# StavrosOrf/EV2Gym

Measured on AMD Instinct MI355X. Metric: env-steps/sec (envs x chargers x steps); % HBM roofline, higher is better.
Workload: dtype f64; 1 GPU; cfg2: V2GProfitPlusLoads, 50 chargers, 1 transformer, uniform[-1,1] actions; envs_per_gpu=4096, scenario_pool_per_gpu=32768, scenario_pool_order=sorted by busy window inside every window of envs_per_gpu scenarios, chargers=50, transformers=1, steps_per_episode=112, obs_dim=162, soc_log=True, launch=persistent, actor=none

## Files before the change

### ev2gym_amd/csrc/ev2g_host.hip

```cpp
#include <hip/hip_runtime.h>

#include <algorithm>
#include <cmath>
#include <cstdio>
#include <cstring>
#include <array>
#include <map>
#include <string>
#include <vector>

#include "../../include/ev2g.h"
#include "ev2g_device.h"
#include "ev2g_load_host.h"
#include "ev2g_step_v2.h"
#include "ev2g_step_wave.h"
#include "ev2g_step_big.h"
#include "ev2g_mlp.h"
#include "ev2g_comm.h"
#include "ev2g_refill.h"
#include "ev2g_heuristic.h"
#include "ev2g_link.h"
#include "ev2g_grid.h"
#include "ev2g_wrap.h"
#include "ev2g_ac.h"
// ... 124 lines not shown
    std::string big_reason;
    size_t lds_big = 0;
    BigArgs big_args{};
    bool no_full = false, no_wide = false;
    bool no_strided = false;
    std::map<ClsKey, int> cls_map;
    ClsRec *d_cls_rec = nullptr;
    std::vector<double> cs_vk_host;
    std::vector<int> cs_ph_host;
    std::vector<double> cs_imax_host;
    int load_gen = 0;
    int last_spec = -1;
    double *d_stats_inl = nullptr;
    const char *inl_shape_reason = "";
    bool inl_stats = false, no_inl_stats = false;
    int last_stats_route = -1;
    const char *inl_reason = "";
    const char *stats_reason = "";
    const char *general_reason = "";
    bool pow2_dt = false;
    std::string kernel_name;
    std::string fallback_reason;
    int current_step = 0;
    long long state_epoch = 0;
    size_t lds_bytes = 0;
    hipEvent_t ev0s[EV2G_EV_RING] = {}, ev1s[EV2G_EV_RING] = {};
    int ev_slot = 0;
    bool ev_valid[EV2G_EV_RING] = {};
    unsigned fused_attr_mask = 0;
    long long ev_calls = 0;
// ... 171 lines not shown
    if (h->own_stream) (void)hipStreamDestroy(h->stream);
    delete h;
}

int ev2g_n_envs(const ev2g_handle *h) { return h ? h->E : 0; }
int ev2g_n_ports(const ev2g_handle *h) { return h ? h->P : 0; }
int ev2g_obs_dim(const ev2g_handle *h) { return h ? h->D : 0; }
int ev2g_n_steps(const ev2g_handle *h) { return h ? h->T : 0; }
int ev2g_current_step(const ev2g_handle *h) { return h ? h->current_step : 0; }
const char *ev2g_kernel_name(const ev2g_handle *h) { return (h && h->loaded) ? h->kernel_name.c_str() : ""; }
const char *ev2g_fallback_reason(const ev2g_handle *h) { return (h && h->loaded) ? h->fallback_reason.c_str() : ""; }
const char *ev2g_big_kernel_reason(const ev2g_handle *h) { return (h && h->loaded) ? h->big_reason.c_str() : ""; }
int ev2g_last_launch_specialisation(const ev2g_handle *h) { return (h && h->loaded) ? h->last_spec : -1; }
int ev2g_last_stats_route(const ev2g_handle *h) { return (h && h->loaded) ? h->last_stats_route : -1; }
const char *ev2g_last_stats_reason(const ev2g_handle *h) { return (h && h->loaded && h->last_stats_route == 0) ? h->stats_reason : ""; }
const char *ev2g_last_launch_general_reason(const ev2g_handle *h) { return (h && h->loaded && h->last_spec == 0) ? h->general_reason : ""; }

static const char *kStatNames[EV2G_N_STATS] = {
    "total_ev_served", "total_profits", "total_energy_charged", "total_energy_discharged",
    "average_user_satisfaction", "power_tracker_violation", "tracking_error", "energy_tracking_error",
    "energy_user_satisfaction", "std_energy_user_satisfaction", "min_energy_user_satisfaction",
    "total_steps_min_emergency_battery_capacity_violation", "total_transformer_overload",
    "battery_degradation", "battery_degradation_calendar", "battery_degradation_cycling", "total_reward"};
const char *ev2g_stat_name(int i) { return (i >= 0 && i < EV2G_N_STATS) ? kStatNames[i] : ""; }

int ev2g_reset_ex(ev2g_handle *h, double *obs, int64_t scenario_offset);

static bool stats_pair(const ev2g_handle *h) {
    const long long per_scn = h->sess_cap > 0 ? (long long)h->sess_cap : (h->S + h->M - 1) / std::max(h->M, 1);
    return (h->sess_cap > 0 ? per_scn <= 48 : h->S <= (long long)h->M * 24) && h->C <= 32;
// ... 7 lines not shown
    s.E = E; s.M = M; s.T = T; s.C = C; s.npc = npc; s.P = P; s.R = R; s.D = D; s.ND = std::max(p.ND, 1); s.dt = p.dt;
    s.reward_kind = h->cfg.reward_kind; s.state_kind = sk; s.flags = h->cfg.flags; s.cost_kind = h->cfg.cost_kind; s.n_lut = p.n_lut;
    s.het = p.het ? 1 : 0;
    h->block = p.het ? 0 : (P <= 256) ? 256 : (P <= 512) ? 512 : (P <= 1024) ? 1024 : 0;
    const int blk = h->block ? h->block : EV2G_BLOCK;
    s.G = std::max(1, blk / P);
    s.G = std::min(s.G, E);
    h->fallback_reason.clear();
    if (P < 2 || P > 64) h->fallback_reason = "ports per env outside 2..64";
    else if (R != 1) h->fallback_reason = "more than one transformer";
    else if (npc != 1) h->fallback_reason = "multi-port chargers";
    if (p.het) h->fallback_reason = "chargers with different port counts (topology file)";
    h->wave_path = h->fallback_reason.empty();
    h->no_full = sw.no_full; h->no_wide = sw.no_wide; h->last_spec = -1;
    h->no_strided = sw.no_strided;
    h->no_inl_stats = sw.no_inl_stats; h->inl_stats = false; h->last_stats_route = -1; h->inl_reason = "no step launch since the scenarios were loaded";
    h->state_epoch += 1;
    if (h->wave_path) {
        const unsigned long long lim = 1ull << 32;
        const unsigned long long biggest = std::max({(unsigned long long)E * P * 8, (unsigned long long)E * D * 8,
                                                     (unsigned long long)M * (T + 1) * 60 * 8, (unsigned long long)p.SD * sizeof(SessRec),
                                                     (unsigned long long)M * T * 64, (unsigned long long)E * T * 8 * 3, (unsigned long long)M * P * 8, (unsigned long long)E * P * sizeof(PortLine),
                                                     (h->cfg.flags & EV2G_FLAG_LOG_SOC) ? (unsigned long long)E * T * P * 8 : 0ull,
                                                     (h->cfg.flags & EV2G_FLAG_LOG_CS_HISTORY) ? (unsigned long long)T * E * C * 8 : 0ull});
        if (biggest >= lim) { h->wave_path = false; h->fallback_reason = "an array of the batch reaches 4 GiB (32-bit byte offsets)"; }
    }
    if (h->wave_path) {
        h->wave_epw = 64 / P; h->wave_es = P;
        s.G = (EV2G_WAVE_BLOCK / 64) * h->wave_epw;
    }
// ... 245 lines not shown
    EV2G_SETP(v2p.ss_afap, h->d_ss_afap);
    int ex = 0;
    v2p.pow2_dt = (std::frexp(h->scn.sixty_over_dt, &ex) == 0.5 && h->scn.sixty_over_dt * h->scn.dt_over_60 == 1.0) ? 1 : 0;
    h->pow2_dt = v2p.pow2_dt != 0;
    return upload(h, h->st_allocs, &v2p, 1, &h->d_v2p);
}

static int load_decide_inl_stats(ev2g_handle *h) {
    h->d_stats_inl = nullptr;
    const char *why = "";
    if (h->no_inl_stats) why = "EV2G_NO_INLAUNCH_STATS is set";
    else if (!h->wave_path || !(h->cfg.flags & EV2G_FLAG_LOG_SOC)) why = "the step kernel is not ev2g_step_wave with the SoC log";
    else if (h->wave_epw != 1 || stats_pair(h)) why = "several envs per wavefront (the in-launch phase computes one env per wavefront, like the statistics kernel at this shape)";
    else if (h->lds_bytes < ev2g_inl_stats_lds_bytes()) why = "the step kernel's LDS is smaller than the phase's blocks";
    h->inl_shape_reason = why;
    if (!why[0]) {
        int rc = 0;
        if ((rc = dalloc(h, h->st_allocs, (size_t)h->E * EV2G_N_STATS, &h->d_stats_inl))) return rc;
        double *p = h->d_stats_inl;
        HIPCHK(h, hipMemcpy((char *)h->d_v2p + offsetof(V2P, stats_inl), &p, sizeof p, hipMemcpyHostToDevice));
    }
    return EV2G_OK;
}

int ev2g_load_scenarios(ev2g_handle *h, const ev2g_scenario_batch *b) {
    if (!h || !b) return fail(h, EV2G_ERR_ARG, "ev2g_load_scenarios: null argument");
    (void)hipSetDevice(h->device);
    const LoadSwitches sw = load_switches_from_env();
    LoadPlan plan;
    V2P v2p;
// ... 107 lines not shown
    io.reward = r.reward.p; io.r_stride = r.reward.stride;
    io.done = r.done.p; io.d_stride = r.done.stride;
    io.mask = r.mask.p; io.m_stride = r.mask.stride;
    io.scn_off = (int)h->scn_off;
    io.scn_stride = (auto_reset == EV2G_AUTO_RESET_NEXT) ? h->E % h->M : 0;
    io.step0 = (int)step0;
    io.log_soc = (h->cfg.flags & EV2G_FLAG_LOG_SOC) ? 1 : 0;
    io.act32 = r.actions.p ? nullptr : h->extras.actions_f32;
    io.obs32 = (h->extras.obs_f32 && h->extras.obs_f32_step_stride == 0) ? h->extras.obs_f32 : nullptr;
    return io;
}

static int launch_steps(ev2g_handle *h, const StepIO &io, int t0, int k, int auto_reset) {
    const DevScn &s = h->scn;
    h->inl_stats = false; h->inl_reason = "the step kernel is not ev2g_step_wave"; h->state_epoch += 1;
    if (h->wave_path) {
        const long long lim = 1ll << 32;
        const ev2g_step_extras &x = h->extras;
        if (io.a_stride * 8 >= lim || io.o_stride * 8 >= lim || io.r_stride * 8 >= lim || io.d_stride >= lim || io.m_stride >= lim ||
            x.cost_step_stride * 8 >= lim || x.obs_f32_step_stride * 4 >= lim || io.a_stride < 0 || io.o_stride < 0 || io.r_stride < 0 ||
            io.d_stride < 0 || io.m_stride < 0 || x.cost_step_stride < 0 || x.obs_f32_step_stride < 0)
            return fail(h, EV2G_ERR_ARG, "ev2g_step_n: a step stride is negative or reaches 4 GiB (unsupported by the fast-path kernel)");
        const V2P *pp = (const V2P *)h->d_v2p;
        const DevState &st = h->st;
        const FusedArgs fa0{};
        const WaveArgs wa{s.P, s.T, s.E, s.D, s.M, st.slab_port, st.slab_port_slice, st.hist,
                    st.env_acc, s.cs_pack, (char *)st.line, h->d_step_tab, (char *)st.port_dyn, s.dict, h->wave_epw, h->wave_es};
        const bool f64io = io.actions && io.obs && !x.obs_f32, f32io = !io.actions && io.act32 && !io.obs && io.obs32;
        const bool full0 = (f64io || f32io) && io.reward && io.done && io.mask && !x.cost && !(h->cfg.flags & EV2G_FLAG_LOG_CS_HISTORY) &&
                           !auto_reset && t0 + k <= s.T && std::min(s.reward_kind, 3) != 3 && !h->no_full;
        const bool wide0 = full0 && (h->cfg.flags & EV2G_FLAG_LOG_SOC) && s.P >= 3 && !h->no_wide &&
                           s.P >= (s.state_kind == EV2G_STATE_PUBLIC_PST ? 3 : (s.state_kind == EV2G_STATE_V2G_PROFIT_MAX_LOADS ? 30 : 10));
        const bool strided = io.o_stride != 0 || io.r_stride != 0 || io.d_stride != 0 || io.m_stride != 0;
        const bool str3 = strided && wide0 && f64io && !h->no_strided;
        const bool full = full0 && (!strided || str3), wide = wide0 && full;
        h->last_spec = full ? (str3 ? 3 : (wide ? 2 : 1)) : 0;
        {
            const char *why = "";
            if (!full) {
                if (h->no_full) why = "EV2G_NO_FULL is set (or the batch has more than 4094 efficiency tables)";
                else if (std::min(s.reward_kind, 3) == 3) why = "the reward function is one of the eight selected at run time (only the shipped configs' three are compiled in)";
                else if (h->cfg.flags & EV2G_FLAG_LOG_CS_HISTORY) why = "EV2G_FLAG_LOG_CS_HISTORY (charger histories)";
                else if (x.cost) why = "a cost buffer is registered (ev2g_set_step_extras)";
                else if (auto_reset) why = "auto_reset";
                else if (!(io.reward && io.done && io.mask)) why = "a reward / done / mask output is NULL";
                else if (!(f64io || f32io)) why = "the observation / action buffers are neither the float64 pair nor the float32 hand-over pair (e.g. obs NULL, or a float32 observation copy next to the float64 one)";
                else if (strided) why = "an output step stride is not 0 (strided outputs keep the specialisation only with float64 observations, EV2G_FLAG_LOG_SOC and an env wide enough for the wide instantiation)";
                else why = "the launch would run past the episode end";
            }
            h->general_reason = why;
        }
// ... 370 lines not shown
static bool fused_eligible(const ev2g_handle *h, const ev2g_mlp *m) {
    const DevScn &s = h->scn;
    const bool pst = s.state_kind == EV2G_STATE_PUBLIC_PST;
    return h->wave_path && s.P >= 3 && s.P <= 64 && std::min(s.reward_kind, 3) != 3 && (h->cfg.flags & EV2G_FLAG_LOG_SOC) &&
           !(h->cfg.flags & EV2G_FLAG_LOG_CS_HISTORY) && !h->extras.cost && !h->no_full && !h->no_wide && (pst || (s.D & 1) == 0) &&
           m->s16_ks1 == (pst ? 2 : 6) && m->s16_nt1 == 25 && m->s16_nt2 == 19 && m->s16_nt3 == (pst ? 2 : 4) &&
           (m->s16_nw == 1 || (m->s16_nw == 2 && !std::getenv("EV2G_NO_FUSED_F32"))) &&
           !std::getenv("EV2G_NO_FUSED");
}
static int launch_fused(ev2g_handle *h, const ev2g_mlp *m, int k, const float *obs0, Rows<float> obs, Rows<float> act, Rows<double> reward,
                        Rows<uint8_t> done, Rows<uint8_t> mask) {
    const DevScn &s = h->scn;
    const DevState &st = h->st;
    const long long lim = 1ll << 32;
    h->inl_stats = false; h->inl_reason = "the last launch was a policy-in-the-loop segment (ev2g_rollout / ev2g_collect)"; h->state_epoch += 1;
    if (obs.stride * 4 >= lim || act.stride * 4 >= lim || reward.stride * 8 >= lim || done.stride >= lim || mask.stride >= lim || obs.stride < 0 ||
        act.stride < 0 || reward.stride < 0 || done.stride < 0 || mask.stride < 0)
        return fail(h, EV2G_ERR_ARG, "ev2g_collect / ev2g_rollout: a step stride is negative or reaches 4 GiB");
    StepIO io = make_io(h, StepRows{{nullptr, act.stride}, {nullptr, obs.stride}, reward, done, mask}, 0, 0);
    io.act32 = act.p; io.obs32 = obs.p;
    const int ae = (s.state_kind == EV2G_STATE_PUBLIC_PST && s.P <= 32 && m->s16_nw == 1) ? 2 : 1;
    const WaveArgs wa{s.P, s.T, s.E, s.D, s.M, st.slab_port, st.slab_port_slice, st.hist, st.env_acc, s.cs_pack, (char *)st.line, h->d_step_tab, (char *)st.port_dyn, s.dict, ae, ae == 1 ? s.P : 32};
    FusedArgs fa{};
    fa.m = m->dev; fa.obs0 = obs0;
    const V2P *pp = (const V2P *)h->d_v2p;
    const int nwf = m->s16_nw;
    const size_t lds = ev2g_fused_lds_bytes(ae, nwf);
    const dim3 grid((s.E + 16 * ae - 1) / (16 * ae)), block(EV2G_FUSED_BLOCK);
    const int t0 = h->current_step;
#define EV2G_FUSED_CASE(SK, RK)                                                                                                            \
// ... 1348 lines not shown
```

### ev2gym_amd/csrc/ev2g_load_host.h

```cpp
#pragma once
#include <algorithm>
#include <array>
#include <cmath>
#include <cstdlib>
#include <cstring>
#include <map>
#include <string>
#include <utility>
#include <vector>

#include "../../include/ev2g.h"
#include "ev2g_records.h"

struct LoadSwitches {
    long long pool_session_cap = 0;
    bool no_full = false, no_wide = false, no_strided = false;
    bool no_inl_stats = false;
    bool kernel_v2 = false;
    bool no_dict = false;
    bool no_big = false;
};
inline LoadSwitches load_switches_from_env() {
    LoadSwitches sw;
    if (const char *e = std::getenv("EV2G_POOL_SESSION_CAP")) sw.pool_session_cap = std::atoll(e);
    sw.no_full = std::getenv("EV2G_NO_FULL") != nullptr;
    sw.no_wide = std::getenv("EV2G_NO_WIDE") != nullptr;
    sw.no_strided = std::getenv("EV2G_NO_STRIDED") != nullptr;
    sw.no_inl_stats = std::getenv("EV2G_NO_INLAUNCH_STATS") != nullptr;
    const char *kn = std::getenv("EV2G_KERNEL");
    sw.kernel_v2 = kn && std::string(kn) == "v2";
    sw.no_dict = std::getenv("EV2G_NO_DICT") != nullptr;
    sw.no_big = std::getenv("EV2G_NO_BIG") != nullptr;
    return sw;
}

typedef std::array<uint64_t, 11> ClsKey;
inline int cls_find_or_add(std::map<ClsKey, int> &map, std::vector<ClsRec> &tab, const ClsRec &c) {
    ClsKey k;
    const double f[11] = {c.pacmax, c.tsm, c.gate_ch, c.B, c.rB, c.v, c.rv, c.gate_dis, c.minB, c.emerg, c.pdismax};
    std::memcpy(k.data(), f, sizeof f);
    auto it = map.find(k);
    if (it != map.end()) return it->second;
    if (map.size() >= EV2G_CLS_CAP) return -1;
// ... 372 lines not shown
```

### ev2gym_amd/csrc/ev2g_step_v2.h

```cpp
#pragma once
#include "ev2g_device.h"

#ifdef EV2G_PHASE_TIMING
#define PT_DECL unsigned long long pt_last = __builtin_readcyclecounter(); unsigned long long pt_acc[18] = {0,0,0,0,0,0,0,0,0,0,0,0,0,0,0,0,0,0}; unsigned long long pt_cur[8] = {0,0,0,0,0,0,0,0};
#define PT_MARK(i) { unsigned long long n_ = __builtin_readcyclecounter(); pt_cur[i] += n_ - pt_last; pt_last = n_; }
#define PT_STEP_END(empty) { const int o_ = (empty) ? 8 : 0; for (int i_ = 0; i_ < 8; i_++) { pt_acc[o_ + i_] += pt_cur[i_]; pt_cur[i_] = 0; } pt_acc[16 + ((empty) ? 1 : 0)] += 1; }
#ifndef EV2G_PT_TID
#define EV2G_PT_TID 0
#endif
#define PT_FLUSH if (threadIdx.x == EV2G_PT_TID && S->dbg) { for (int i_ = 0; i_ < 8; i_++) pt_acc[i_] += pt_cur[i_]; for (int i_ = 0; i_ < 18; i_++) S->dbg[(size_t)blockIdx.x * 18 + i_] += pt_acc[i_]; }
#elif defined(EV2G_PHASE_MARKERS)
#define PT_DECL
#define PT_MARK(i) asm volatile("; PHASE_MARK " #i);
#define PT_STEP_END(empty)
#define PT_FLUSH
#else
#define PT_DECL
#define PT_MARK(i)
#define PT_STEP_END(empty)
#define PT_FLUSH
#endif

__device__ __forceinline__ void lds_barrier() { asm volatile("s_waitcnt lgkmcnt(0)\n\ts_barrier" ::: "memory"); }

// ... 96 lines not shown
    EV2G_GP(const double) head_tab;
    EV2G_GP(const SessRec) rec; EV2G_GP(const SessTail) tail; EV2G_GP(const int) ss_lut;
    EV2G_GP(const SessDyn) sess_dyn; EV2G_GP(const ClsRec) cls_rec;
    EV2G_GP(PortLine) line;
    EV2G_GP(double) cs_sat_sum; EV2G_GP(int) cs_served;
    EV2G_GP(double) cs_profits; EV2G_GP(double) cs_e_ch; EV2G_GP(double) cs_e_dis;
    EV2G_GP(double) cs_power_hist; EV2G_GP(double) cs_cur_hist; EV2G_GP(double) cs_power_now; EV2G_GP(double) cs_cur_now;
    EV2G_GP(double) env_acc; EV2G_GP(int) env_fault;
    EV2G_GP(double) hist; EV2G_GP(double) tr_power_now;
    EV2G_GP(double) sess_final_cap; EV2G_GP(double) port_energy; EV2G_GP(double) port_current;
    EV2G_GP(double) soc_log; EV2G_GP(double) sess_abs_e;
    EV2G_GP(unsigned long long) dbg;
    EV2G_GP(const int) scn_sess; EV2G_GP(const int) scn_sess_end; EV2G_GP(const int) ss_slot; EV2G_GP(const int) ss_tarr; EV2G_GP(const int) ss_tdep;
    EV2G_GP(const double) ss_B; EV2G_GP(const double) ss_afap;
    EV2G_GP(double) stats_inl;
    EV2G_GP(double) x_cost; long long x_c_stride;
    EV2G_GP(float) x_obs32; long long x_o32_stride;
    EV2G_GP(const float) x_act32;
};

inline void ev2g_v2_fill_params(V2P &p, const DevScn &s, const DevState &st) {
    p.E = s.E; p.M = s.M; p.cost_kind = s.cost_kind; p.T = s.T; p.C = s.C; p.npc = s.npc; p.P = s.P; p.R = s.R; p.D = s.D; p.G = s.G; p.dt = s.dt;
    p.reward_kind = s.reward_kind; p.state_kind = s.state_kind; p.n_lut = s.n_lut;
    p.sixty_over_dt = s.sixty_over_dt; p.dt_over_60 = s.dt_over_60;
    p.rdt = 1.0 / (double)s.dt; p.dt_fdiv = fabs(fma((double)s.dt, p.rdt, -1.0)) <= 0x1p-54 ? 1 : 0;
    EV2G_SETP(p.x_cost, (double *)nullptr); EV2G_SETP(p.x_obs32, (float *)nullptr); EV2G_SETP(p.x_act32, (const float *)nullptr);
    p.x_c_stride = 0; p.x_o32_stride = 0;
    p.pow2_dt = 0; EV2G_SETP(p.head_tab, (const double *)nullptr);
    EV2G_SETP(p.step_tab, (const double *)nullptr);
    EV2G_SETP(p.slab_port, st.slab_port); p.slab_port_slice = st.slab_port_slice;
    EV2G_SETP(p.slab_hist, st.slab_hist); EV2G_SETP(p.slab_sess, st.slab_sess);
    p.sess_slice = (unsigned long long)(st.sess_abs_e ? (st.sess_abs_e - st.slab_sess) : 0) * 8ull;
#define CPS(f) EV2G_SETP(p.f, s.f);
#define CPT(f) EV2G_SETP(p.f, st.f);
    CPS(slot_cs) CPS(slot_port) CPS(slot_obs) CPS(cs_slot0) CPS(tr_seg) CPS(tr_obs) CPS(port_first) CPS(port_first_win)
    CPS(cs_imax) CPS(cs_imin) CPS(cs_dmin) CPS(cs_dmax_abs) CPS(cs_maxp) CPS(cs_minp)
    CPS(price_ch) CPS(price_dis) CPS(setpoint) CPS(tr_infl) CPS(tr_solar) CPS(tr_base) CPS(tr_maxp) CPS(tr_minp)
    CPS(win_tab) CPS(lut) CPS(rec) CPS(tail) CPS(ss_lut) CPS(sess_dyn) CPS(cls_rec)
    CPS(scn_sess) CPS(scn_sess_end) CPS(ss_slot) CPS(ss_tarr) CPS(ss_tdep) CPS(ss_B)
    EV2G_SETP(p.ss_afap, (const double *)nullptr); EV2G_SETP(p.stats_inl, (double *)nullptr);
    CPT(line) CPT(cs_sat_sum) CPT(cs_served)
    CPT(cs_profits) CPT(cs_e_ch) CPT(cs_e_dis) CPT(cs_power_hist) CPT(cs_cur_hist) CPT(cs_power_now) CPT(cs_cur_now)
    CPT(env_acc) CPT(env_fault) CPT(hist) CPT(tr_power_now)
    CPT(sess_final_cap) CPT(port_energy) CPT(port_current) CPT(soc_log) CPT(sess_abs_e) CPT(dbg)
#undef CPS
#undef CPT
}

__host__ __device__ inline size_t ev2g_v2_lds_bytes(int NS, int NT, int G, int R) {
    return sizeof(double) * ((size_t)(EV2G_NQ + 7) * NS + (size_t)EV2G_NQ * NT + (size_t)EV2G_NQ * G + (size_t)NT +
                             (size_t)G * 9) +
           sizeof(int) * (6 * (size_t)NS + 2 * (size_t)R + 1 + 4);
}

#define V2C(x, c) (SPEC ? (c) : (x))
// ... 581 lines not shown
```

### ev2gym_amd/csrc/ev2g_step_wave.h

```cpp
#pragma once
#include <type_traits>
#include "ev2g_step_v2.h"
#include "ev2g_mlp.h"

#define EV2G_WAVE_BLOCK 256

__host__ __device__ inline size_t ev2g_wave_lds_bytes(int envs_per_group, int block = EV2G_WAVE_BLOCK) {
    const size_t NS = (size_t)block;
    return sizeof(double) * (EV2G_NQ * (NS + 8) + 7 * NS + 7 * (size_t)envs_per_group + 4 * 64) + sizeof(int) * (6 * NS + 8);
}
#define EV2G_INL_STATS_NK 12
#define EV2G_INL_STATS_LK 16
__host__ __device__ inline size_t ev2g_inl_stats_lds_bytes(int block = EV2G_WAVE_BLOCK) { return (size_t)block * EV2G_INL_STATS_LK * sizeof(double); }
#define EV2G_FUSED_BLOCK 1024
#define EV2G_FUSED_SX 200
#define EV2G_FUSED_RING 10
#define EV2G_FUSED_RING2 7

#define EV2G_FUSED_SXF 196
#define EV2G_FUSED_RINGF 4
__host__ __device__ inline size_t ev2g_fused_lds_bytes(int envs_per_wave = 1, int weight_terms = 1) {
    if (weight_terms > 1)
        return ev2g_wave_lds_bytes(EV2G_FUSED_BLOCK / 64 * envs_per_wave, EV2G_FUSED_BLOCK) + (size_t)16 * EV2G_FUSED_SXF * 4;
    return ev2g_wave_lds_bytes(EV2G_FUSED_BLOCK / 64 * envs_per_wave, EV2G_FUSED_BLOCK) + (size_t)16 * EV2G_FUSED_SX * 2 + (size_t)(25 + 19 + 4) * 16 * 4;
// ... 125 lines not shown
    float *lbias = (float *)(bufX + 16 * EV2G_FUSED_SX);
    float *act_lds = (float *)s_amps;
    uint16_t *bufH1 = (uint16_t *)stage, *bufH2 = bufH1 + 16 * AE * MC::SH1;
    constexpr int FSXF = EV2G_FUSED_SXF;
    float *bufXf = (float *)(cnt + 8);
    static_assert(NWF == 1 || (3 * 16 * MC::SH1 * 2 <= 5 * RS * 8 && EV2G_NQ == 8 && FKS1 * 32 <= 256), "the input rows' bf16 terms live in staging rows 5..7, behind H1's three copies");
    static_assert(NWF == 1 || (FKS1 * 32 + 4 <= FSXF && (3 * MC::SH1 + 2 * MC::SH2) * 16 * 2 <= EV2G_NQ * (EV2G_FUSED_BLOCK + 8) * 8 && MC::SH2 * 16 * 2 <= 16 * FSXF * 4), "float32 policy buffers");
    static_assert(AE * MC::SX <= EV2G_FUSED_SX && MC::NB <= (25 + 19 + 4) * 16 && 16 * AE * (MC::SH1 + MC::SH2) * 2 <= EV2G_NQ * (EV2G_FUSED_BLOCK + 8) * 8, "policy buffers");
    constexpr int ACT_AS = (AE == 1) ? 128 : 64;
    const int tid = threadIdx.x, wv = tid >> 6, lane = tid & 63;
    const bool log_soc = WIDE ? true : (S->soc_log != nullptr);
    const bool log_cs = FULL ? false : (S->cs_profits != nullptr);
    const double dtd = (double)S->dt, sixty_over_dt = S->sixty_over_dt, dt_over_60 = S->dt_over_60;
    const bool pow2_dt = S->pow2_dt != 0;

    const int elw = lane / ES;
    const int q = (ACT && AE == 1) ? lane : lane - elw * ES;
    const int e = (ACT && AE == 1) ? e0 + wv : e0 + wv * EPW + elw;
    const bool valid = (elw < EPW) && (q < P) && (e < E);
    const bool hcopy = ACT && AE == 1 && !valid && e < E && lane < 32;
    const int g = valid ? e * P + q : 0;
    const int ocol = (SK == 1) ? 3 + 3 * q : (SK == 0 ? 62 + 2 * q : 22 + 2 * q);
    const int cs = valid ? q : 0;
    int t = t0;
    const bool head = valid && q == 0;
    const int elg = wv * EPW + elw;
    const int arow = (AE == 1) ? wv : min(elg, 16 * AE - 1);
    auto xput2 = [&](int col, float a, float b) __attribute__((always_inline)) {
        if (NWF > 1) *(float2 *)(bufXf + arow * FSXF + col) = make_float2(a, b);
        else *(uint32_t *)(bufX + arow * FSX + col) = ev2g_pack_bf16(a, b);
// ... 183 lines not shown
        d2v pf_h0 = {0.0, 0.0}, pf_h1 = {0.0, 0.0};
        constexpr int NHEAD = (SK == 1) ? 0 : (SK == 0 ? 60 : 20);
        constexpr int NPAIR = NHEAD / 2;
        if (!out) {
        } else if (SK == 1) {
            pf_ob0 = ldg32_nt<double>(S->step_tab, eT64 + (unsigned)min(sstep, T - 1) * 64u + 40u);
        } else {
            const unsigned h8 = FULL ? hb_head + (unsigned)sstep * (unsigned)(NHEAD * 8) : (unsigned)((scn * (T + 1) + sstep) * NHEAD) * 8u;
            pf_h0 = ldg32_nt<d2v>(S->head_tab, h8 + (unsigned)min(q_l, NPAIR - 1) * 16u);
            if (!WIDE && P < NPAIR) pf_h1 = ldg32_nt<d2v>(S->head_tab, h8 + (unsigned)min(q_l + P, NPAIR - 1) * 16u);
        }
        bool occ = false;
        double cap_before = 0.0;
        int ta_a = EV2G_INT_MAX, td_a = -1;
        const bool wave_live = !FULL || EPW != 1 || __ballot(valid && ((r_ta <= t && t <= r_td) || r_ta == sstep)) != 0ull;
        if (valid && wave_live) {
            int ta = FULL ? r_ta : s_ta[tid_l], td = FULL ? r_td : s_td[tid_l];
            double cap_b = s_cap[tid_l], c_thr = s_cst[0 * 64 + q_l], c_dmin = s_cst[1 * 64 + q_l];
            asm volatile("s_waitcnt lgkmcnt(0)" : "+v"(ta), "+v"(td), "+v"(cap_b), "+v"(c_thr), "+v"(c_dmin));
            ta_a = ta; td_a = td;
            occ = (ta <= t) && (t <= td);
            if (log_soc && occ) cap_before = cap_b;
            double a = occ ? a_cur : 0.0;
            a = (a > 1.0) ? 1.0 : ((a < -1.0) ? -1.0 : a);
            const double n5 = rint(a * 100000.0), q5 = n5 * (1.0 / 100000.0);
            const double x = fma(fma(-q5, 100000.0, n5), 1.0 / 100000.0, q5);
            const double ac = x * c_imax, ad = x * c_dmaxabs;
            const double amps_c = (ac < c_thr) ? 0.0 : ac, amps_d = (ad > c_dmin - 0.01) ? c_dmin : ad;
            const double amps = (x > 0.0) ? amps_c : ((x < 0.0) ? amps_d : 0.0);
            s_amps[tid_l] = amps;
// ... 15 lines not shown
            static_assert(offsetof(SessRec, B) == 40 && offsetof(SessRec, rB) == 48 && offsetof(SessRec, cap0) == 112 && offsetof(SessRec, potc) == 120 && sizeof(SessTail) == 16 &&
                          offsetof(SessTail, nt_arr) == 8, "SessRec / SessTail layout");
            pf_c2 = ldg32<d2v_a8>(S->rec, sse * (unsigned)sizeof(SessRec) + 40u); pf_c7 = ldg32<d2v>(S->rec, sse * (unsigned)sizeof(SessRec) + 112u);
            pf_tl = ldg32<i4v>(S->tail, sse * 16u);
            pf_d0 = ldg32<d2v>(S->sess_dyn, sse * 32u); pf_d1 = ldg32<i4v>(S->sess_dyn, sse * 32u + 16u);
        }
#if defined(EV2G_PHASE_TIMING) && defined(EV2G_PT_OUTER)
        PT_MARK(0)
#else
        PT_MARK(6)
#endif
        lds_barrier();
        PT_MARK(1)

        const int nch = cntk[0], ndis = cntk[1];
        if (nch + ndis != 0) {
        __builtin_amdgcn_s_setprio(3);
        {
            const int nchp = (nch + 63) & ~63;
            for (int i = tid_l; i < nchp + ndis; i += BLOCK) {
                int h = -1;
                if (i < nch) h = items[i];
                else if (i >= nchp) h = items[NS - 1 - (i - nchp)];
                if (h >= 0) {
                    const double amps_h = s_amps[h];
                    const int dw_h = s_dirty[h];
                    const int lut_id = ((dw_h >> 8) & LUTMASK) - 1;
                    const int li = (lut_id >= 0) ? ev_lut_index(lut_id, amps_h) : -1;
                    double lut_raw = ldg32<double>(S->lut, (unsigned)max(li, 0) * 8u);
                    const unsigned r8 = ((FULL && wa.dict) ? (unsigned)dw_h >> 20 : (unsigned)s_ss[h]) * (unsigned)sizeof(SessRec);
// ... 320 lines not shown
                ri.user = esum[2]; ri.tr0_maxp = pf_maxp;
                reward = ev2g_reward(S->reward_kind, ri);
            } else {
                reward = costs - over100 - esum[2];
            }
            const double n0 = ea0 + reward, n1 = ea1 + costs, n2 = ea2 + esum[4], n3 = ea3 + esum[5], n4 = ea4 + esum[6];
            ea[0] = n0; ea[1] = n1; ea[2] = n2; ea[3] = n3; ea[4] = n4; ea[5] = potn;
            if (RK == 3) ea[6] = ea5;
            if (FULL && out) { stg32<double>(rew_run, e8, reward); stg32<uint8_t>(done_run, (unsigned)e_l, (sstep >= T) ? 1 : 0); }
            if (!FULL && io.reward) stg32<double>(io.reward + (long long)kk * io.r_stride, e8, reward);
            if (!FULL && io.done) stg32<uint8_t>(io.done + (long long)kk * io.d_stride, (unsigned)e_l, (sstep >= T) ? 1 : 0);
            if (!FULL && S->x_cost)
                stg32<double>(S->x_cost + (long long)(io.step0 + kk) * S->x_c_stride, e8, (S->cost_kind == 2) ? costs : 100.0 * over + esum[2]);
            if (sstep >= T || last_step) {
                const unsigned a8 = (unsigned)e_l * 64u;
                stg32<d2v>(env_acc, a8, (d2v){n0, n1});
                stg32<d2v>(env_acc, a8 + 16u, (d2v){n2, n3});
                stg32<double>(env_acc, a8 + 32u, n4);
            }
        }
        if ((valid || hcopy) && ((F32 && out) || (!FULL && obs32))) {
            const unsigned o4 = FULL ? hb_obs_env : (unsigned)(e_l * D) * 4u;
            if (SK == 1) {
                if (q_l == 0) {
                    const float h0 = (float)((double)sstep / (double)T), h1 = (float)((sstep < T) ? pf_ob0 : 0.0), h2 = (float)usage;
                    stg32<float>(obs32, o4, h0);
                    stg32<float>(obs32, o4 + 4u, h1);
                    stg32<float>(obs32, o4 + 8u, h2);
                    if (ACT && NWF > 1) { bufXf[arow * FSXF] = h0; bufXf[arow * FSXF + 1] = h1; bufXf[arow * FSXF + 2] = h2; }
                    else
                    if (ACT) {
                        *(uint32_t *)(bufX + arow * FSX) = ev2g_pack_bf16(h0, h1);
                        bufX[arow * FSX + 2] = (uint16_t)ev2g_pack_bf16(h2, 0.f);
// ... 80 lines not shown
```

### ev2gym_amd/engine.py

```python
from __future__ import annotations

import ctypes as C
import os
import warnings
from typing import Optional

import numpy as np

from . import _abi
from .scenario import ScenarioBatch

_LIB_PATH = os.path.join(os.path.dirname(os.path.abspath(__file__)), "libev2g_hip.so")
_lib = None


class EngineError(RuntimeError):
    def __init__(self, code, msg):
        super().__init__(f"[ev2g {code}] {msg}")
        self.code = code


def load_library(path: Optional[str] = None):
    global _lib
    if _lib is not None:
# ... 14 lines not shown
        "ev2g_create": (C.c_int, [C.POINTER(_abi.ConfigC), C.POINTER(vp)]),
        "ev2g_destroy": (None, [vp]),
        "ev2g_last_error": (C.c_char_p, [vp]),
        "ev2g_load_scenarios": (C.c_int, [vp, C.POINTER(_abi.ScenarioBatchC)]),
        "ev2g_n_envs": (C.c_int, [vp]), "ev2g_n_scenarios": (C.c_int, [vp]), "ev2g_n_ports": (C.c_int, [vp]), "ev2g_obs_dim": (C.c_int, [vp]),
        "ev2g_n_steps": (C.c_int, [vp]), "ev2g_current_step": (C.c_int, [vp]),
        "ev2g_reset": (C.c_int, [vp, vp]),
        "ev2g_reset_ex": (C.c_int, [vp, vp, i64]),
        "ev2g_scenario_offset": (i64, [vp]),
        "ev2g_set_step_extras": (C.c_int, [vp, C.POINTER(_abi.StepExtrasC)]),
        "ev2g_kernel_name": (C.c_char_p, [vp]),
        "ev2g_last_launch_specialisation": (C.c_int, [vp]),
        "ev2g_last_launch_general_reason": (C.c_char_p, [vp]),
        "ev2g_last_stats_route": (C.c_int, [vp]),
        "ev2g_last_stats_reason": (C.c_char_p, [vp]),
        "ev2g_fallback_reason": (C.c_char_p, [vp]),
        "ev2g_big_kernel_reason": (C.c_char_p, [vp]),
        "ev2g_step": (C.c_int, [vp, vp, vp, vp, vp, vp]),
        "ev2g_step_n": (C.c_int, [vp, C.c_int, C.c_int, vp, i64, vp, i64, vp, i64, vp, i64, vp, i64, C.c_int]),
        "ev2g_check_faults": (C.c_int, [vp, C.POINTER(i32)]),
        "ev2g_get_stats": (C.c_int, [vp, vp]),
        "ev2g_get_stats_reset": (C.c_int, [vp, vp, vp, C.c_int64]),
        "ev2g_get_stats_reset_f32": (C.c_int, [vp, vp, vp, C.c_int64]),
        "ev2g_reset_f32": (C.c_int, [vp, vp, C.c_int64]),
        "ev2g_collect": (C.c_int, [vp, vp, C.c_int, vp]),
        "ev2g_heuristic_create": (C.c_int, [vp, C.c_int, C.POINTER(vp)]),
        "ev2g_heuristic_destroy": (None, [vp, vp]),
        "ev2g_heuristic_actions": (C.c_int, [vp, vp, vp]),
        "ev2g_heuristic_run": (C.c_int, [vp, vp, C.c_int, vp, i64, vp, i64, vp, i64, vp, i64, vp, i64]),
        "ev2g_link_create": (C.c_int, [vp, dbl, dbl, C.c_uint64, C.c_uint64, vp, vp, C.POINTER(vp)]),
# ... 66 lines not shown
        "ev2g_gen_table": (C.c_int, [C.c_int, C.c_int, C.POINTER(C.c_double), C.c_int]),
    }
    for name, (res, args) in protos.items():
        fn = getattr(L, name)
        fn.restype = res
        fn.argtypes = args
    if L.ev2g_abi_version() != _abi.ABI_VERSION:
        raise EngineError(-1, "libev2g_hip.so ABI version mismatch")
    _lib = L
    return L


EXPORTED_SYMBOLS = [
    "ev2g_abi_version", "ev2g_create", "ev2g_destroy", "ev2g_last_error", "ev2g_load_scenarios", "ev2g_n_envs",
    "ev2g_n_scenarios", "ev2g_n_ports", "ev2g_obs_dim", "ev2g_n_steps", "ev2g_current_step", "ev2g_reset", "ev2g_reset_ex",
    "ev2g_scenario_offset", "ev2g_set_step_extras", "ev2g_kernel_name", "ev2g_last_launch_specialisation", "ev2g_last_launch_general_reason", "ev2g_last_stats_route", "ev2g_last_stats_reason", "ev2g_fallback_reason", "ev2g_big_kernel_reason", "ev2g_step", "ev2g_step_n",
    "ev2g_check_faults", "ev2g_get_stats", "ev2g_get_stats_reset", "ev2g_get_stats_reset_f32", "ev2g_reset_f32", "ev2g_collect", "ev2g_stat_name", "ev2g_peek", "ev2g_malloc", "ev2g_free",
    "ev2g_memcpy_h2d", "ev2g_memcpy_d2h", "ev2g_host_malloc", "ev2g_host_free", "ev2g_synchronize", "ev2g_fill_uniform", "ev2g_host_uniform",
    "ev2g_last_step_n_kernel_ms", "ev2g_step_n_kernel_ms_back", "ev2g_mlp_create", "ev2g_mlp_create_ex", "ev2g_mlp_destroy", "ev2g_mlp_forward", "ev2g_rollout",
    "ev2g_rollout_graph_launches", "ev2g_comm_get_unique_id", "ev2g_comm_init", "ev2g_comm_destroy", "ev2g_comm_world_size", "ev2g_comm_gathers", "ev2g_gather_stats",
    "ev2g_pool_refill", "ev2g_pool_refill_overflows", "ev2g_pool_session_capacity", "ev2g_gen_default_config", "ev2g_generate", "ev2g_gen_batch", "ev2g_gen_free", "ev2g_gen_table",
    "ev2g_heuristic_create", "ev2g_heuristic_destroy", "ev2g_heuristic_actions", "ev2g_heuristic_run",
    "ev2g_link_create", "ev2g_link_destroy", "ev2g_link_reset_state", "ev2g_link_actions", "ev2g_link_observe", "ev2g_link_obs_f32",
    "ev2g_link_run", "ev2g_link_rollout",
    "ev2g_grid_create", "ev2g_grid_destroy", "ev2g_grid_solve", "ev2g_grid_run",
    "ev2g_grid_state_attach", "ev2g_grid_state_dim", "ev2g_grid_observe", "ev2g_grid_run_observed", "ev2g_grid_rollout", "ev2g_grid_get_stats",
    "ev2g_wrap_create", "ev2g_wrap_destroy", "ev2g_wrap_reset_state", "ev2g_wrap_actions", "ev2g_wrap_run", "ev2g_wrap_rollout",
    "ev2g_ac_create", "ev2g_ac_destroy", "ev2g_ac_seed", "ev2g_ac_set_log_std", "ev2g_ac_set_weights", "ev2g_ac_forward", "ev2g_ac_act",
    "ev2g_ac_collect", "ev2g_ac_host_normal", "ev2g_gae", "ev2g_host_gae"]


# ... 75 lines not shown
    @property
    def kernel_name(self) -> str:
        return (self._lib.ev2g_kernel_name(self._h) or b"").decode()

    @property
    def last_launch_specialisation(self) -> int:
        return int(self._lib.ev2g_last_launch_specialisation(self._h))

    @property
    def last_stats_route(self) -> int:
        return int(self._lib.ev2g_last_stats_route(self._h))

    @property
    def last_stats_reason(self) -> str:
        return (self._lib.ev2g_last_stats_reason(self._h) or b"").decode()

    @property
    def fallback_reason(self) -> str:
        return (self._lib.ev2g_fallback_reason(self._h) or b"").decode()

    @property
    def big_kernel_reason(self) -> str:
        return (self._lib.ev2g_big_kernel_reason(self._h) or b"").decode()

    @property
    def scenario_offset(self) -> int:
        return int(self._lib.ev2g_scenario_offset(self._h))

    def set_extras(self, cost=None, cost_stride=0, obs_f32=None, obs_f32_stride=0, actions_f32=None):
        self._extras_keep = (cost, obs_f32, actions_f32)
# ... 431 lines not shown
```

### include/ev2g.h

```cpp
#ifndef EV2G_H
#define EV2G_H

#include <stddef.h>
#include <stdint.h>

#ifdef __cplusplus
extern "C" {
#endif

#define EV2G_ABI_VERSION 4

#define EV2G_REWARD_PROFITMAX_TRPENALTY_USERINCENTIVES 0
#define EV2G_REWARD_SQUARED_TRACKING_ERROR 1
#define EV2G_REWARD_PROFIT_MAXIMIZATION 2
#define EV2G_REWARD_SQTR_TRPENALTY_USERINCENTIVES 3
#define EV2G_REWARD_SQUARED_TRACKING_ERROR_PENALTY 4
#define EV2G_REWARD_SIMPLE 5
#define EV2G_REWARD_MINIMIZE_TRACKER_SURPLUS 6
#define EV2G_REWARD_V2G_COSTS_SIMPLE 7
#define EV2G_REWARD_V2G_PROFITMAX 8
#define EV2G_REWARD_V2G_PROFITMAX_V2 9
#define EV2G_REWARD_PST_V2G_PROFITMAX_V2 10
#define EV2G_N_REWARDS 11
#define EV2G_STATE_V2G_PROFIT_MAX_LOADS 0
// ... 123 lines not shown
    int64_t cost_step_stride;
    float *obs_f32;
    int64_t obs_f32_step_stride;
    const float *actions_f32;
} ev2g_step_extras;
int ev2g_set_step_extras(ev2g_handle *h, const ev2g_step_extras *x);

int ev2g_current_step(const ev2g_handle *h);
const char *ev2g_kernel_name(const ev2g_handle *h);
const char *ev2g_fallback_reason(const ev2g_handle *h);
const char *ev2g_big_kernel_reason(const ev2g_handle *h);
int ev2g_last_launch_specialisation(const ev2g_handle *h);
const char *ev2g_last_launch_general_reason(const ev2g_handle *h);
int ev2g_last_stats_route(const ev2g_handle *h);
const char *ev2g_last_stats_reason(const ev2g_handle *h);
int ev2g_check_faults(ev2g_handle *h, int32_t *first_bad_env);

int ev2g_get_stats(ev2g_handle *h, double *stats);
int ev2g_get_stats_reset(ev2g_handle *h, double *stats, double *obs, int64_t scenario_offset);
int ev2g_get_stats_reset_f32(ev2g_handle *h, double *stats, float *obs32, int64_t scenario_offset);
int ev2g_reset_f32(ev2g_handle *h, float *obs32, int64_t scenario_offset);
const char *ev2g_stat_name(int i);

#define EV2G_COMM_ID_BYTES 128
int ev2g_comm_get_unique_id(void *id_out);
int ev2g_comm_init(ev2g_handle *h, const void *id, int rank, int world_size);
void ev2g_comm_destroy(ev2g_handle *h);
int ev2g_comm_world_size(const ev2g_handle *h);
long long ev2g_comm_gathers(const ev2g_handle *h);
int ev2g_gather_stats(ev2g_handle *h, double *stats_all);
// ... 198 lines not shown
```

Measured before the change: 1.168 billion env-steps/s.

## Fast-forward idle stretches of wave kernel steps when no EV is connected

Adds a fast-forward path to the wavefront step kernel. When a wavefront's env has no connected EV until the next arrival, it computes the trivial rewards and history for up to 64 steps at once and jumps ahead, instead of running the full per-step pipeline. A per-group counter records the skipped steps and stretches, and an environment switch disables the path. This adds LDS traffic and a barrier for the lookahead, plus extra register pressure in the kernel.

After: 1.224 billion env-steps/s, median of 6. 1.05x the previous value.

```diff
diff --git a/ev2gym_amd/csrc/ev2g_host.hip b/ev2gym_amd/csrc/ev2g_host.hip
--- a/ev2gym_amd/csrc/ev2g_host.hip
+++ b/ev2gym_amd/csrc/ev2g_host.hip
@@ -162,6 +162,8 @@
     double *d_stats_inl = nullptr;
     const char *inl_shape_reason = "";
     bool inl_stats = false, no_inl_stats = false;
+    unsigned long long *d_ff_count = nullptr;
+    bool no_fast_forward = false, ff_launch = false;
     int last_stats_route = -1;
     const char *inl_reason = "";
     const char *stats_reason = "";
@@ -363,6 +365,20 @@
 int ev2g_last_launch_specialisation(const ev2g_handle *h) { return (h && h->loaded) ? h->last_spec : -1; }
 int ev2g_last_stats_route(const ev2g_handle *h) { return (h && h->loaded) ? h->last_stats_route : -1; }
 const char *ev2g_last_stats_reason(const ev2g_handle *h) { return (h && h->loaded && h->last_stats_route == 0) ? h->stats_reason : ""; }
+int ev2g_last_launch_fast_forwarded(ev2g_handle *h, int64_t *steps, int64_t *stretches) {
+    if (!h || !h->loaded) return fail(h, EV2G_ERR_STATE, "ev2g_last_launch_fast_forwarded: no scenarios loaded");
+    int64_t n = 0, m = 0;
+    if (h->ff_launch) {
+        (void)hipSetDevice(h->device);
+        std::vector<unsigned long long> c((size_t)h->scn.n_groups);
+        HIPCHK(h, hipMemcpyAsync(c.data(), h->d_ff_count, sizeof(unsigned long long) * c.size(), hipMemcpyDeviceToHost, h->stream));
+        HIPCHK(h, hipStreamSynchronize(h->stream));
+        for (unsigned long long v : c) { n += (int64_t)(v & 0xffffffffull); m += (int64_t)(v >> 32); }
+    }
+    if (steps) *steps = n;
+    if (stretches) *stretches = m;
+    return EV2G_OK;
+}
 const char *ev2g_last_launch_general_reason(const ev2g_handle *h) { return (h && h->loaded && h->last_spec == 0) ? h->general_reason : ""; }
 
 static const char *kStatNames[EV2G_N_STATS] = {
@@ -400,6 +416,7 @@
     h->wave_path = h->fallback_reason.empty();
     h->no_full = sw.no_full; h->no_wide = sw.no_wide; h->last_spec = -1;
     h->no_strided = sw.no_strided;
+    h->no_fast_forward = sw.no_fast_forward; h->ff_launch = false;
     h->no_inl_stats = sw.no_inl_stats; h->inl_stats = false; h->last_stats_route = -1; h->inl_reason = "no step launch since the scenarios were loaded";
     h->state_epoch += 1;
     if (h->wave_path) {
@@ -675,6 +692,13 @@
     else if (h->wave_epw != 1 || stats_pair(h)) why = "several envs per wavefront (the in-launch phase computes one env per wavefront, like the statistics kernel at this shape)";
     else if (h->lds_bytes < ev2g_inl_stats_lds_bytes()) why = "the step kernel's LDS is smaller than the phase's blocks";
     h->inl_shape_reason = why;
+    h->d_ff_count = nullptr;
+    if (h->wave_path && h->wave_epw == 1 && !h->no_fast_forward) {
+        int rc = 0;
+        if ((rc = dalloc(h, h->st_allocs, (size_t)h->scn.n_groups, &h->d_ff_count))) return rc;
+        unsigned long long *p = h->d_ff_count;
+        HIPCHK(h, hipMemcpy((char *)h->d_v2p + offsetof(V2P, ff_count), &p, sizeof p, hipMemcpyHostToDevice));
+    }
     if (!why[0]) {
         int rc = 0;
         if ((rc = dalloc(h, h->st_allocs, (size_t)h->E * EV2G_N_STATS, &h->d_stats_inl))) return rc;
@@ -812,6 +836,7 @@
 static int launch_steps(ev2g_handle *h, const StepIO &io, int t0, int k, int auto_reset) {
     const DevScn &s = h->scn;
     h->inl_stats = false; h->inl_reason = "the step kernel is not ev2g_step_wave"; h->state_epoch += 1;
+    h->ff_launch = false;
     if (h->wave_path) {
         const long long lim = 1ll << 32;
         const ev2g_step_extras &x = h->extras;
@@ -833,6 +858,7 @@
         const bool str3 = strided && wide0 && f64io && !h->no_strided;
         const bool full = full0 && (!strided || str3), wide = wide0 && full;
         h->last_spec = full ? (str3 ? 3 : (wide ? 2 : 1)) : 0;
+        h->ff_launch = full && !str3 && f64io && k > 1 && h->d_ff_count != nullptr && s.state_kind != EV2G_STATE_PUBLIC_PST;
         {
             const char *why = "";
             if (!full) {
@@ -1233,6 +1259,7 @@
     const DevState &st = h->st;
     const long long lim = 1ll << 32;
     h->inl_stats = false; h->inl_reason = "the last launch was a policy-in-the-loop segment (ev2g_rollout / ev2g_collect)"; h->state_epoch += 1;
+    h->ff_launch = false;
     if (obs.stride * 4 >= lim || act.stride * 4 >= lim || reward.stride * 8 >= lim || done.stride >= lim || mask.stride >= lim || obs.stride < 0 ||
         act.stride < 0 || reward.stride < 0 || done.stride < 0 || mask.stride < 0)
         return fail(h, EV2G_ERR_ARG, "ev2g_collect / ev2g_rollout: a step stride is negative or reaches 4 GiB");
diff --git a/ev2gym_amd/csrc/ev2g_load_host.h b/ev2gym_amd/csrc/ev2g_load_host.h
--- a/ev2gym_amd/csrc/ev2g_load_host.h
+++ b/ev2gym_amd/csrc/ev2g_load_host.h
@@ -16,6 +16,7 @@
     long long pool_session_cap = 0;
     bool no_full = false, no_wide = false, no_strided = false;
     bool no_inl_stats = false;
+    bool no_fast_forward = false;
     bool kernel_v2 = false;
     bool no_dict = false;
     bool no_big = false;
@@ -27,6 +28,7 @@
     sw.no_wide = std::getenv("EV2G_NO_WIDE") != nullptr;
     sw.no_strided = std::getenv("EV2G_NO_STRIDED") != nullptr;
     sw.no_inl_stats = std::getenv("EV2G_NO_INLAUNCH_STATS") != nullptr;
+    sw.no_fast_forward = std::getenv("EV2G_NO_FAST_FORWARD") != nullptr;
     const char *kn = std::getenv("EV2G_KERNEL");
     sw.kernel_v2 = kn && std::string(kn) == "v2";
     sw.no_dict = std::getenv("EV2G_NO_DICT") != nullptr;
diff --git a/ev2gym_amd/csrc/ev2g_step_v2.h b/ev2gym_amd/csrc/ev2g_step_v2.h
--- a/ev2gym_amd/csrc/ev2g_step_v2.h
+++ b/ev2gym_amd/csrc/ev2g_step_v2.h
@@ -134,6 +134,7 @@
     EV2G_GP(const int) scn_sess; EV2G_GP(const int) scn_sess_end; EV2G_GP(const int) ss_slot; EV2G_GP(const int) ss_tarr; EV2G_GP(const int) ss_tdep;
     EV2G_GP(const double) ss_B; EV2G_GP(const double) ss_afap;
     EV2G_GP(double) stats_inl;
+    EV2G_GP(unsigned long long) ff_count;
     EV2G_GP(double) x_cost; long long x_c_stride;
     EV2G_GP(float) x_obs32; long long x_o32_stride;
     EV2G_GP(const float) x_act32;
@@ -158,7 +159,7 @@
     CPS(price_ch) CPS(price_dis) CPS(setpoint) CPS(tr_infl) CPS(tr_solar) CPS(tr_base) CPS(tr_maxp) CPS(tr_minp)
     CPS(win_tab) CPS(lut) CPS(rec) CPS(tail) CPS(ss_lut) CPS(sess_dyn) CPS(cls_rec)
     CPS(scn_sess) CPS(scn_sess_end) CPS(ss_slot) CPS(ss_tarr) CPS(ss_tdep) CPS(ss_B)
-    EV2G_SETP(p.ss_afap, (const double *)nullptr); EV2G_SETP(p.stats_inl, (double *)nullptr);
+    EV2G_SETP(p.ss_afap, (const double *)nullptr); EV2G_SETP(p.stats_inl, (double *)nullptr); EV2G_SETP(p.ff_count, (unsigned long long *)nullptr);
     CPT(line) CPT(cs_sat_sum) CPT(cs_served)
     CPT(cs_profits) CPT(cs_e_ch) CPT(cs_e_dis) CPT(cs_power_hist) CPT(cs_cur_hist) CPT(cs_power_now) CPT(cs_cur_now)
     CPT(env_acc) CPT(env_fault) CPT(hist) CPT(tr_power_now)
diff --git a/ev2gym_amd/csrc/ev2g_step_wave.h b/ev2gym_amd/csrc/ev2g_step_wave.h
--- a/ev2gym_amd/csrc/ev2g_step_wave.h
+++ b/ev2gym_amd/csrc/ev2g_step_wave.h
@@ -4,6 +4,9 @@
 #include "ev2g_mlp.h"
 
 #define EV2G_WAVE_BLOCK 256
+#ifndef EV2G_FF_N_MIN
+#define EV2G_FF_N_MIN 1
+#endif
 
 __host__ __device__ inline size_t ev2g_wave_lds_bytes(int envs_per_group, int block = EV2G_WAVE_BLOCK) {
     const size_t NS = (size_t)block;
@@ -163,6 +166,18 @@
     const double dtd = (double)S->dt, sixty_over_dt = S->sixty_over_dt, dt_over_60 = S->dt_over_60;
     const bool pow2_dt = S->pow2_dt != 0;
 
+#if defined(EV2G_PHASE_TIMING)
+    constexpr bool FFW = false;
+#else
+    constexpr bool FFW = F64 && LSO && !ACT && RK != 3 && SK != 1 && BLOCK == EV2G_WAVE_BLOCK;
+#endif
+    unsigned short *ffx = (unsigned short *)(cnt + 4);
+    int ff_lim_v = 0;
+    int ff_next_v = -1;
+    if (FFW && EPW == 1 && k_steps > 1 && S->ff_count != nullptr) {
+        ff_lim_v = k_steps - 1;
+        if (tid == 0) stg32<unsigned long long>(S->ff_count, (unsigned)blockIdx.x * 8u, 0ull);
+    }
     const int elw = lane / ES;
     const int q = (ACT && AE == 1) ? lane : lane - elw * ES;
     const int e = (ACT && AE == 1) ? e0 + wv : e0 + wv * EPW + elw;
@@ -376,6 +391,19 @@
         double cap_before = 0.0;
         int ta_a = EV2G_INT_MAX, td_a = -1;
         const bool wave_live = !FULL || EPW != 1 || __ballot(valid && ((r_ta <= t && t <= r_td) || r_ta == sstep)) != 0ull;
+        if (FFW) asm volatile("" : "+v"(ff_lim_v), "+v"(ff_next_v));
+        if (FFW && EPW == 1 && __builtin_amdgcn_readfirstlane(ff_lim_v) != 0) {
+            int ff_next = __builtin_amdgcn_readfirstlane(ff_next_v);
+            if (wave_live) ff_next = t;
+            else if (ff_next <= t) {
+                int m = (valid && r_ta > sstep) ? r_ta : EV2G_INT_MAX;
+#pragma unroll
+                for (int o = 32; o > 0; o >>= 1) m = min(m, __shfl_xor(m, o));
+                ff_next = __builtin_amdgcn_readfirstlane(m) - 1;
+            }
+            ff_next_v = ff_next;
+            if (lane_l == 0) ffx[4 * (kk & 1) + (tid_l >> 6)] = (unsigned short)min(ff_next - t, 0xffff);
+        }
         if (valid && wave_live) {
             int ta = FULL ? r_ta : s_ta[tid_l], td = FULL ? r_td : s_td[tid_l];
             double cap_b = s_cap[tid_l], c_thr = s_cst[0 * 64 + q_l], c_dmin = s_cst[1 * 64 + q_l];
@@ -421,6 +449,61 @@
         PT_MARK(1)
 
         const int nch = cntk[0], ndis = cntk[1];
+        if (FFW) asm volatile("" : "+v"(ff_lim_v));
+        const int ff_lim = (FFW && EPW == 1) ? __builtin_amdgcn_readfirstlane(ff_lim_v) : 0;
+        if (FFW && ff_lim != 0) {
+            const uint2 fx = *(const uint2 *)(ffx + 4 * (kk & 1));
+            const unsigned f01 = min(fx.x & 0xffffu, fx.x >> 16), f23 = min(fx.y & 0xffffu, fx.y >> 16);
+            const int n = __builtin_amdgcn_readfirstlane(min(min((int)min(f01, f23), 64), ff_lim - kk));
+            if (n >= EV2G_FF_N_MIN) {
+                lds_barrier();
+                const int ew = __builtin_amdgcn_readfirstlane(e_l);
+                const int Tf = S->T;
+                int bx = (int)blockIdx.x;
+                asm volatile("" : "+s"(bx));
+                if (ew < S->E) {
+                    const int ts = t + lane_l;
+                    const unsigned row = (unsigned)__builtin_amdgcn_readfirstlane(hb_step) + (unsigned)min(ts, Tf - 1) * 64u;
+                    const d2v tr0 = ldg32_nt<d2v>(S->step_tab, row + 16u), tr1 = ldg32_nt<d2v>(S->step_tab, row + 32u);
+                    double *ea = eacc + (tid_l >> 6) * 7;
+                    double n0 = ea[0], n1 = ea[1], n2 = ea[2], n3 = ea[3], n4 = ea[4];
+                    const double pot_t = ea[5];
+                    const double usage = 0.0, costs = 0.0, user = 0.0;
+                    const double tr_power = tr0.x + usage;
+                    const double over = (tr_power > tr0.y + 0.0001 || tr_power < tr1.x - 0.0001) ? fabs(tr_power - tr0.y) : 0.0;
+                    double reward;
+                    if (RK == 1) {
+                        const double pp = (lane_l == 0) ? pot_t : 0.0;
+                        const double mn = (pp < tr1.y) ? pp : tr1.y;
+                        const double d = mn - usage;
+                        reward = -(d * d);
+                    } else if (RK == 2) {
+                        reward = costs - user;
+                    } else {
+                        reward = costs - 100.0 * over - user;
+                    }
+                    if (lane_l < n) {
+                        const unsigned h8 = (unsigned)(ew * Tf + ts) * 24u;
+                        stg32<double>(S->hist, h8, usage);
+                        stg32<double>(S->hist, h8 + 16u, over);
+                        if (ts + 1 < Tf) stg32<double>(S->hist, h8 + 32u, 0.0);
+                    }
+                    const int r_lo = __double2loint(reward), r_hi = __double2hiint(reward);
+                    for (int j = 0; j < n; j++)
+                        n0 += __hiloint2double(__builtin_amdgcn_readlane(r_hi, j), __builtin_amdgcn_readlane(r_lo, j));
+                    n1 += 0.0; n2 += 0.0; n3 += 0.0; n4 += 0.0;
+                    if (lane_l == 0) { ea[0] = n0; ea[1] = n1; ea[2] = n2; ea[3] = n3; ea[4] = n4; ea[5] = 0.0; }
+                }
+                if (tid_l == 0)
+                    __hip_atomic_fetch_add((unsigned long long __attribute__((address_space(1))) *)((gptr)S->ff_count + (unsigned)bx * 8u),
+                                           (1ull << 32) | (unsigned long long)n, __ATOMIC_RELAXED, __HIP_MEMORY_SCOPE_AGENT);
+                a_next = ldg32_nt<double>(act_run + (long long)(n - 1) * io.a_stride, (unsigned)gc * 8u);
+                act_run += (long long)(n - 1) * io.a_stride;
+                t += n;
+                kk += n - 1;
+                continue;
+            }
+        }
         if (nch + ndis != 0) {
         __builtin_amdgcn_s_setprio(3);
         {
@@ -771,9 +854,15 @@
                 stg32<double>(S->x_cost + (long long)(io.step0 + kk) * S->x_c_stride, e8, (S->cost_kind == 2) ? costs : 100.0 * over + esum[2]);
             if (sstep >= T || last_step) {
                 const unsigned a8 = (unsigned)e_l * 64u;
-                stg32<d2v>(env_acc, a8, (d2v){n0, n1});
-                stg32<d2v>(env_acc, a8 + 16u, (d2v){n2, n3});
-                stg32<double>(env_acc, a8 + 32u, n4);
+                if (FFW) {
+                    stg32<d2v>(S->env_acc, a8, (d2v){n0, n1});
+                    stg32<d2v>(S->env_acc, a8 + 16u, (d2v){n2, n3});
+                    stg32<double>(S->env_acc, a8 + 32u, n4);
+                } else {
+                    stg32<d2v>(env_acc, a8, (d2v){n0, n1});
+                    stg32<d2v>(env_acc, a8 + 16u, (d2v){n2, n3});
+                    stg32<double>(env_acc, a8 + 32u, n4);
+                }
             }
         }
         if ((valid || hcopy) && ((F32 && out) || (!FULL && obs32))) {
diff --git a/ev2gym_amd/engine.py b/ev2gym_amd/engine.py
--- a/ev2gym_amd/engine.py
+++ b/ev2gym_amd/engine.py
@@ -52,6 +52,7 @@
         "ev2g_last_launch_general_reason": (C.c_char_p, [vp]),
         "ev2g_last_stats_route": (C.c_int, [vp]),
         "ev2g_last_stats_reason": (C.c_char_p, [vp]),
+        "ev2g_last_launch_fast_forwarded": (C.c_int, [vp, C.POINTER(C.c_int64), C.POINTER(C.c_int64)]),
         "ev2g_fallback_reason": (C.c_char_p, [vp]),
         "ev2g_big_kernel_reason": (C.c_char_p, [vp]),
         "ev2g_step": (C.c_int, [vp, vp, vp, vp, vp, vp]),
@@ -148,7 +149,7 @@
 EXPORTED_SYMBOLS = [
     "ev2g_abi_version", "ev2g_create", "ev2g_destroy", "ev2g_last_error", "ev2g_load_scenarios", "ev2g_n_envs",
     "ev2g_n_scenarios", "ev2g_n_ports", "ev2g_obs_dim", "ev2g_n_steps", "ev2g_current_step", "ev2g_reset", "ev2g_reset_ex",
-    "ev2g_scenario_offset", "ev2g_set_step_extras", "ev2g_kernel_name", "ev2g_last_launch_specialisation", "ev2g_last_launch_general_reason", "ev2g_last_stats_route", "ev2g_last_stats_reason", "ev2g_fallback_reason", "ev2g_big_kernel_reason", "ev2g_step", "ev2g_step_n",
+    "ev2g_scenario_offset", "ev2g_set_step_extras", "ev2g_kernel_name", "ev2g_last_launch_specialisation", "ev2g_last_launch_general_reason", "ev2g_last_stats_route", "ev2g_last_stats_reason", "ev2g_last_launch_fast_forwarded", "ev2g_fallback_reason", "ev2g_big_kernel_reason", "ev2g_step", "ev2g_step_n",
     "ev2g_check_faults", "ev2g_get_stats", "ev2g_get_stats_reset", "ev2g_get_stats_reset_f32", "ev2g_reset_f32", "ev2g_collect", "ev2g_stat_name", "ev2g_peek", "ev2g_malloc", "ev2g_free",
     "ev2g_memcpy_h2d", "ev2g_memcpy_d2h", "ev2g_host_malloc", "ev2g_host_free", "ev2g_synchronize", "ev2g_fill_uniform", "ev2g_host_uniform",
     "ev2g_last_step_n_kernel_ms", "ev2g_step_n_kernel_ms_back", "ev2g_mlp_create", "ev2g_mlp_create_ex", "ev2g_mlp_destroy", "ev2g_mlp_forward", "ev2g_rollout",
@@ -254,6 +255,12 @@
     @property
     def last_stats_reason(self) -> str:
         return (self._lib.ev2g_last_stats_reason(self._h) or b"").decode()
+
+    @property
+    def last_launch_fast_forwarded(self):
+        n, m = C.c_int64(0), C.c_int64(0)
+        self._check(self._lib.ev2g_last_launch_fast_forwarded(self._h, C.byref(n), C.byref(m)))
+        return int(n.value), int(m.value)
 
     @property
     def fallback_reason(self) -> str:
diff --git a/include/ev2g.h b/include/ev2g.h
--- a/include/ev2g.h
+++ b/include/ev2g.h
@@ -161,6 +161,7 @@
 const char *ev2g_last_launch_general_reason(const ev2g_handle *h);
 int ev2g_last_stats_route(const ev2g_handle *h);
 const char *ev2g_last_stats_reason(const ev2g_handle *h);
+int ev2g_last_launch_fast_forwarded(ev2g_handle *h, int64_t *steps, int64_t *stretches);
 int ev2g_check_faults(ev2g_handle *h, int32_t *first_bad_env);
 
 int ev2g_get_stats(ev2g_handle *h, double *stats);
```
